# JediZ/PDE-based-image-processing

Measured on AMD Instinct MI355X. Metric: SOR iterations/sec (3840x2160 flow), higher is better.
Workload: dtype f32

## Files before the change

pde-based-image-processing_amd/csrc/pdeip_ctx.hip:

```cpp
#include "pdeip_ctx.hpp"

namespace pdeip {

Context g;
thread_local ThreadState tls;

int set_err(int code, const char *fmt, ...)
{
    va_list ap;
    va_start(ap, fmt);
    vsnprintf(tls.err, sizeof tls.err, fmt, ap);
    va_end(ap);
    return code;
}

SweepTimer::SweepTimer(hipStream_t stream) : s(stream)
{
    if (!g.profile) return;
    std::lock_guard<std::mutex> lock(g.ev_mutex);
    if (g.n_ev >= Context::MAX_EV) return;
    if (g.n_ev == g.n_ev_created) {
        if (hipEventCreate(&g.ev[g.n_ev][0]) != hipSuccess || hipEventCreate(&g.ev[g.n_ev][1]) != hipSuccess) return;
        g.n_ev_created++;
    }
    slot = g.n_ev++;
    (void)hipEventRecord(g.ev[slot][0], s);
}
void SweepTimer::stop(int launches)
{
    if (slot < 0) return;
    (void)hipEventRecord(g.ev[slot][1], s);
    g.ev_launches[slot] = launches;
}

static void latch_abort(DeviceState *d)
{
    if (!d->ws[WS_CTL] || !d->persist_used) return;
    unsigned word = 0;
    if (hipDeviceSynchronize() == hipSuccess && hipMemcpy(&word, d->ws[WS_CTL], sizeof word, hipMemcpyDeviceToHost) == hipSuccess && word != 0)
        d->abort_latched = true;
}

DeviceState *cur_dev()
{
    if (tls.dev_slot >= 0 && tls.dev_slot < MAX_DEVICES) return &g.devs[tls.dev_slot];
    int dev = 0;
// ... 306 lines not shown
```

pde-based-image-processing_amd/csrc/pdeip_ctx.hpp:

```cpp
#pragma once
#include "../../include/pdeip.h"

#include <hip/hip_runtime.h>

#include <atomic>
#include <cstdarg>
#include <cstdio>
#include <cstdlib>
#include <cstring>
#include <map>
#include <mutex>
#include <vector>

namespace pdeip {

enum { WS_AUX0 = 0, WS_AUX1, WS_PING, WS_ARENA, WS_CTL, WS_ORDER, WS_ALR, WS_ALR_T, WS_TV, WS_SMALL, WS_MAIL, WS_PACK, WS_DRIVER, WS_LEX, WS_LS, WS_NSLOT };

constexpr int MAX_DEVICES = 16;

struct DeviceState {
    int device = -1;
    void *ws[WS_NSLOT] = {};
    size_t ws_bytes[WS_NSLOT] = {};
    int order_B = 0, order_T = 0, order_affine = -1;
    int num_cus = 0;
    bool persist_used = false;
    bool abort_latched = false;
    std::map<const void *, size_t> lds_opt_in;
    std::map<const void *, int> resident_waves;
    hipStream_t worker_stream = nullptr;
    void reset_caches()
    {
        order_B = order_T = 0;
        order_affine = -1;
        persist_used = false;
    }
};

struct ThreadState {
    char err[512] = "";
    int last_launches = 0;
    int dev_slot = -1;
};
extern thread_local ThreadState tls;

struct Context {
    int mode = PDEIP_MODE_EXACT_ORDER;
    std::atomic<int> ws_generation{0};
    int rb_tj = 0;
    bool env_read = false;
    int ngroup = 1;
    int group[MAX_DEVICES] = {0};
    DeviceState devs[MAX_DEVICES];
    bool profile = false;
    static constexpr int MAX_EV = 4096;
    hipEvent_t ev[MAX_EV][2];
    int ev_launches[MAX_EV];
// ... 12 lines not shown

#define RC(expr)             \
    do {                     \
        int rc_ = (expr);    \
        if (rc_) return rc_; \
    } while (0)

#define NONNULL(who, p)                                                                                \
    do {                                                                                               \
        if ((p) == nullptr) return ::pdeip::set_err(PDEIP_ERR_ARG, "%s: argument '%s' is NULL", who, #p); \
    } while (0)

struct SweepTimer {
    hipStream_t s;
    int slot = -1;
    explicit SweepTimer(hipStream_t stream);
    void stop(int launches);
};

DeviceState *cur_dev();
int ws_get(int slot, size_t bytes, float **out);
int ensure_lds(const void *kernel, size_t bytes);
int resident_waves(const void *kernel, int block_threads, int waves_per_block);

int check_dims(const char *who, int nrows, int ncols, int nframes);
int check_mode(const char *who, int mode);
int check_solver(const char *who, int solver);
inline bool aligned16(const void *p) { return (reinterpret_cast<uintptr_t>(p) & 15u) == 0; }
int env_int(const char *name, int dflt);
int check_deriv_dims(const char *who, int nrows, int ncols, int nframes);
int pick_rb_tj(int nrows, int ncols);
int copy_d2d(hipStream_t s, float *dst, const float *src, size_t n);
inline dim3 pixel_grid(int nrows, int ncols, int nz) { return dim3((unsigned)((nrows + 255) / 256), (unsigned)ncols, (unsigned)nz); }
// ... 23 lines not shown
```

pde-based-image-processing_amd/csrc/pdeip_line.hip:

```cpp
#include "pdeip_ctx.hpp"

#include "pdeip_alr.hpp"

using namespace pdeip;

static int check_alr_line(const char *, int, int, int) { return PDEIP_OK; }

struct AlrFactors {
    float *cp[2][2], *dv[2][2];
};

template <class Mdl, bool VERT, int MODE>
static int zebra3_launch(hipStream_t s, const typename Mdl::Ctx &q, float *x, float *cp, float *dv, float *dp, int nrows, int ncols, int nframes,
                         int first, int lastc, int lstep, float omega)
{
    RC(ensure_lds(reinterpret_cast<const void *>(&k_alr_zebra3<Mdl, VERT, MODE>), Z3_LDS_BYTES));
    const int count = (lastc - first) / lstep + 1;
    hipLaunchKernelGGL((k_alr_zebra3<Mdl, VERT, MODE>), dim3((unsigned)((count + ZB_LW - 1) / ZB_LW), (unsigned)nframes), dim3(ZB_THREADS),
                       Z3_LDS_BYTES, s, q, x, cp, dv, dp, nrows, ncols, (size_t)nrows * ncols, first, lastc, lstep, omega);
    tls.last_launches++;
    HIPCHK(hipGetLastError());
    return PDEIP_OK;
}

template <class Mdl>
static int alr_factor(hipStream_t s, const typename Mdl::Ctx *q, const typename Mdl::Ctx *qt, int nch, int nrows, int ncols, int nframes,
                      AlrFactors *f)
{
    const size_t fs = (size_t)nrows * ncols, plane = fs * nframes;
    float *base;
    RC(ws_get(WS_ALR, plane * 8 * sizeof(float), &base));
    const int lo = Mdl::INTERIOR_LINES ? 1 : 0;
    for (int c = 0; c < nch; c++)
// ... 30 lines not shown
static int alr_lex_pass(hipStream_t s, const typename Mdl::Ctx *q, float *const *x, const AlrFactors &f, const int *order,
                        int nch, int nrows, int ncols, int nframes, bool vertical, float omega)
{
    const int lo = Mdl::INTERIOR_LINES ? 1 : 0;
    const int hi = (vertical ? ncols : nrows) - 1 - lo;
    const int n = vertical ? nrows : ncols;
    const size_t fs = (size_t)nrows * ncols;
    const int d = vertical ? 0 : 1;
    const size_t line_bytes = (size_t)n * sizeof(float4);
    if (line_bytes > 160 * 1024) {
        float *g = nullptr;
        RC(ws_get(WS_LEX, line_bytes * nframes, &g));
        for (int c = 0; c < nch; c++) {
            AlrChains<Mdl, 1> ch;
            ch.c[0] = AlrChain<Mdl>{q[order[c]], x[order[c]], f.cp[order[c]][d], f.dv[order[c]][d]};
            if (vertical) hipLaunchKernelGGL((k_alr_lex<Mdl, 1, true, true>), dim3((unsigned)nframes), dim3(ALR_LEX_THREADS), 0, s, ch, nrows, ncols, fs, lo, hi, omega, reinterpret_cast<float4 *>(g));
            else hipLaunchKernelGGL((k_alr_lex<Mdl, 1, false, true>), dim3((unsigned)nframes), dim3(ALR_LEX_THREADS), 0, s, ch, nrows, ncols, fs, lo, hi, omega, reinterpret_cast<float4 *>(g));
            tls.last_launches++;
        }
        HIPCHK(hipGetLastError());
        return PDEIP_OK;
    }
    if (nch == 2 && 2 * line_bytes <= 160 * 1024) {
        AlrChains<Mdl, 2> ch;
        for (int c = 0; c < 2; c++) ch.c[c] = AlrChain<Mdl>{q[order[c]], x[order[c]], f.cp[order[c]][d], f.dv[order[c]][d]};
        if (2 * line_bytes > 64 * 1024)
            RC(ensure_lds(vertical ? reinterpret_cast<const void *>(&k_alr_lex<Mdl, 2, true>) : reinterpret_cast<const void *>(&k_alr_lex<Mdl, 2, false>), 2 * line_bytes));
        if (vertical) hipLaunchKernelGGL((k_alr_lex<Mdl, 2, true>), dim3((unsigned)nframes), dim3(ALR_LEX_THREADS), 2 * line_bytes, s, ch, nrows, ncols, fs, lo, hi, omega);
        else hipLaunchKernelGGL((k_alr_lex<Mdl, 2, false>), dim3((unsigned)nframes), dim3(ALR_LEX_THREADS), 2 * line_bytes, s, ch, nrows, ncols, fs, lo, hi, omega);
        tls.last_launches++;
    } else {
        if (line_bytes > 64 * 1024)
            RC(ensure_lds(vertical ? reinterpret_cast<const void *>(&k_alr_lex<Mdl, 1, true>) : reinterpret_cast<const void *>(&k_alr_lex<Mdl, 1, false>), line_bytes));
        for (int c = 0; c < nch; c++) {
            AlrChains<Mdl, 1> ch;
            ch.c[0] = AlrChain<Mdl>{q[order[c]], x[order[c]], f.cp[order[c]][d], f.dv[order[c]][d]};
            if (vertical) hipLaunchKernelGGL((k_alr_lex<Mdl, 1, true>), dim3((unsigned)nframes), dim3(ALR_LEX_THREADS), line_bytes, s, ch, nrows, ncols, fs, lo, hi, omega);
            else hipLaunchKernelGGL((k_alr_lex<Mdl, 1, false>), dim3((unsigned)nframes), dim3(ALR_LEX_THREADS), line_bytes, s, ch, nrows, ncols, fs, lo, hi, omega);
            tls.last_launches++;
        }
    }
    HIPCHK(hipGetLastError());
    return PDEIP_OK;
}

template <class Mdl>
static int alr_zebra_pass(hipStream_t s, const typename Mdl::Ctx &q, float *x, const float *cpf, const float *dvf, int nrows, int ncols,
                          int nframes, bool vertical, float omega)
{
    const int lo = Mdl::INTERIOR_LINES ? 1 : 0;
    const int hi = (vertical ? ncols : nrows) - 1 - lo;
    const size_t fs = (size_t)nrows * ncols;
    float *cp, *dp;
    RC(ws_get(WS_AUX0, fs * nframes * sizeof(float), &cp));
    RC(ws_get(WS_AUX1, fs * nframes * sizeof(float), &dp));
    for (int colour = 0; colour < 2; colour++) {
        const int first = lo + (((lo & 1) != colour) ? 1 : 0);
        if (first > hi) continue;
        const int lastc = hi - (((hi & 1) != colour) ? 1 : 0);
        {
            if (cpf) {
                if (vertical) RC((zebra3_launch<Mdl, true, ZB_APPLY>(s, q, x, const_cast<float *>(cpf), const_cast<float *>(dvf), dp, nrows, ncols, nframes, first, lastc, 2, omega)));
                else RC((zebra3_launch<Mdl, false, ZB_APPLY>(s, q, x, const_cast<float *>(cpf), const_cast<float *>(dvf), dp, nrows, ncols, nframes, first, lastc, 2, omega)));
                continue;
            }
        }
        const int count = (hi - first) / 2 + 1;
        const dim3 grid((unsigned)((count + 63) / 64), (unsigned)nframes);
        if (vertical) hipLaunchKernelGGL((k_alr_zebra<Mdl, true>), grid, dim3(64), 0, s, q, x, cp, dp, nrows, ncols, fs, lo, hi, colour, omega);
        else hipLaunchKernelGGL((k_alr_zebra<Mdl, false>), grid, dim3(64), 0, s, q, x, cp, dp, nrows, ncols, fs, lo, hi, colour, omega);
        tls.last_launches++;
    }
    HIPCHK(hipGetLastError());
    return PDEIP_OK;
}

template <class Mdl>
static int alr_zebra_pass_pair(hipStream_t s, const typename Mdl::Ctx &qa, float *xa, const float *cpa, const float *dva, const typename Mdl::Ctx &qb,
                               float *xb, const float *cpb, const float *dvb, int nrows, int ncols, int nframes, bool vertical, float omega)
{
    const int lo = Mdl::INTERIOR_LINES ? 1 : 0;
    const int hi = (vertical ? ncols : nrows) - 1 - lo;
    const size_t fs = (size_t)nrows * ncols;
    float *dp;
    RC(ws_get(WS_AUX1, fs * nframes * sizeof(float), &dp));
    if (vertical) RC(ensure_lds(reinterpret_cast<const void *>(&k_alr_zebra3_pair<Mdl, true, ZB_APPLY>), Z3_LDS_BYTES));
    else RC(ensure_lds(reinterpret_cast<const void *>(&k_alr_zebra3_pair<Mdl, false, ZB_APPLY>), Z3_LDS_BYTES));
    for (int colour = 0; colour < 2; colour++) {
        const int first = lo + (((lo & 1) != colour) ? 1 : 0);
        if (first > hi) continue;
        const int lastc = hi - (((hi & 1) != colour) ? 1 : 0);
        const int count = (lastc - first) / 2 + 1;
        const dim3 grid((unsigned)((count + ZB_LW - 1) / ZB_LW), (unsigned)nframes);
        if (vertical)
            hipLaunchKernelGGL((k_alr_zebra3_pair<Mdl, true, ZB_APPLY>), grid, dim3(ZB_THREADS), Z3_LDS_BYTES, s, qa, xa, const_cast<float *>(cpa), const_cast<float *>(dva), qb, xb,
                               const_cast<float *>(cpb), const_cast<float *>(dvb), dp, nrows, ncols, fs, first, lastc, 2, omega);
        else
            hipLaunchKernelGGL((k_alr_zebra3_pair<Mdl, false, ZB_APPLY>), grid, dim3(ZB_THREADS), Z3_LDS_BYTES, s, qa, xa, const_cast<float *>(cpa), const_cast<float *>(dva), qb, xb,
                               const_cast<float *>(cpb), const_cast<float *>(dvb), dp, nrows, ncols, fs, first, lastc, 2, omega);
        tls.last_launches++;
    }
    HIPCHK(hipGetLastError());
    return PDEIP_OK;
}

struct AlrTwin {
    static constexpr int MAXP = 40;
    const float *orig[MAXP];
    float *twin[MAXP];
    int count = 0;
    float *find(const float *p) const
    {
        for (int k = 0; k < count; k++)
// ... 107 lines not shown
                    A.tin[k] = tin[k];
                    A.tout[k] = tout[k];
                }
                float *fbase;
                const size_t fplane = (size_t)nrows * ncols * nframes;
                RC(ws_get(WS_ALR, fplane * 8 * sizeof(float), &fbase));
                for (int c = 0; c < nch; c++)
                    for (int d = 0; d < 2; d++) {
                        A.cp[c][d] = fbase + fplane * (size_t)((c * 2 + d) * 2);
                        A.dv[c][d] = A.cp[c][d] + fplane;
                    }
                A.ntr = ntr; A.nch = nch; A.nrows = nrows; A.ncols = ncols; A.iter = iter; A.omega = omega;
                A.fs = (size_t)nrows * ncols;
                RC(ensure_lds(reinterpret_cast<const void *>(&k_alr_small<Mdl>), lds));
                SweepTimer timer(s);
                hipLaunchKernelGGL(k_alr_small<Mdl>, dim3((unsigned)nframes), dim3(ALR_SMALL_THREADS), lds, s, A);
                timer.stop(iter);
                tls.last_launches++;
                HIPCHK(hipGetLastError());
                return PDEIP_OK;
            }
            tw = AlrTwin{};
        }
    }
    RC(alr_make_twins(s, q, qt, nch, x, xt, nrows, ncols, nframes, &tw));
    AlrFactors f{};
    static const bool zebra1 = env_int("PDEIP_ALR_ZEBRA1", 0) != 0;
    if (mode == PDEIP_MODE_EXACT_ORDER || !zebra1) RC(alr_factor<Mdl>(s, q, qt, nch, nrows, ncols, nframes, &f));
    const bool pair = mode != PDEIP_MODE_EXACT_ORDER && nch == 2 && f.cp[0][0] != nullptr && f.cp[1][0] != nullptr && env_int("PDEIP_ALR_PAIR", 1) != 0;
    SweepTimer timer(s);
    for (int it = 0; it < iter; it++) {
// ... 81 lines not shown
```

pde-based-image-processing_amd/csrc/pdeip_sor5.hip:

```cpp
#include "pdeip_ctx.hpp"

#include "pdeip_models.hpp"
#include "pdeip_pointwise.hpp"
#include "pdeip_sor_exact.hpp"
#include "pdeip_walk_host.hpp"
#include "pdeip_persist_host.hpp"
#include "pdeip_sor_rb.hpp"
#include "pdeip_sor_rbp.hpp"
#include "pdeip_sor_small.hpp"

using namespace pdeip;

namespace {

template <class Mdl>
int pick_rb2_tj(int nrows, int ncols, int nframes, int ntiles_r)
{
    (void)nrows;
    const int forced = g.rb_tj > 0 ? g.rb_tj : env_int("PDEIP_RB_TJ", 0);
    if (forced > 0) return forced < 2 ? 2 : forced;
    const int slots = resident_waves(reinterpret_cast<const void *>(&k_sor_rb<Mdl, true, false, true>), 64 * RB_WAVES_PER_BLOCK, RB_WAVES_PER_BLOCK);
    int best = 12;
    long best_cost = -1;
    for (int tj = 2; tj <= 64; tj++) {
// ... 81 lines not shown
            RC(ws_get(WS_PACK, n * nframes * Mdl::NCF * sizeof(float), &pack));
            hipLaunchKernelGGL(k_pack_coefficients<Mdl>, pixel_grid(nrows, ncols, nframes), dim3(256), 0, s, P, pack, nrows, ncols, n);
            tls.last_launches++;
            const int NC = (nrows - 2 + 63 + EX_CH - 1) / EX_CH;
            const bool walk = env_int("PDEIP_EXACT_WALK", 0) != 0;
            const int W = walk ? walk_width<Mdl>(nrows, ncols, nframes, iter) : 64;
            const int BW = (ncols - 2 + W - 1) / W;
            PersistCtl ctl{};
            RC(persist_prepare(s, BW, iter, nframes, (size_t)nframes * iter * BW * NIT * (size_t)NC * EX_CH * sizeof(unsigned long long), &ctl));
            SweepTimer timer(s);
            if (walk) {
                RC(walk_launch<Mdl>(s, P, pack, ctl, nrows, ncols, BW, iter, NC, nframes, omega, n, W));
            } else {
                constexpr size_t plds = ExactLayout<Mdl>::LDS_BYTES + 16;
                RC(ensure_lds(reinterpret_cast<const void *>(&k_sor_exact_persist<Mdl>), plds));
                hipLaunchKernelGGL(k_sor_exact_persist<Mdl>, dim3((unsigned)(BW * iter * nframes)), dim3(exp_threads<Mdl>()), plds, s, P, pack, ctl, nrows, ncols, BW, iter, NC, nframes, omega, n);
            }
            timer.stop(1);
            tls.last_launches++;
            const int nb = 2 * ncols + 2 * (nrows - 2);
            hipLaunchKernelGGL(k_fill_borders, dim3((nb + 255) / 256, nframes, NIT), dim3(256), 0, s,
                               P.it_out[0], P.it_out[NIT - 1], NIT, nrows, ncols, n);
            tls.last_launches++;
            HIPCHK(hipGetLastError());
            return PDEIP_OK;
        }
        hipLaunchKernelGGL(k_derive<Mdl>, pixel_grid(nrows, ncols, nframes), dim3(256), 0, s, P, aux0, aux1, nrows, ncols, n);
        tls.last_launches++;
        P.cf[Mdl::D0] = aux0;
        P.cf[Mdl::D1] = aux1;
        const dim3 grid((unsigned)(B * iter), (unsigned)nframes);
        constexpr size_t lds = ExactLayout<Mdl>::LDS_BYTES;
        RC(ensure_lds(reinterpret_cast<const void *>(&k_sor_exact<Mdl>), lds));
        SweepTimer timer(s);
        for (int m = 0; m <= last_m; m++) {
            hipLaunchKernelGGL(k_sor_exact<Mdl>, grid, dim3(128), lds, s, P, nrows, ncols, A, B, iter, m, omega, n);
            tls.last_launches++;
        }
        timer.stop(last_m + 1);
        const int nb = 2 * ncols + 2 * (nrows - 2);
        hipLaunchKernelGGL(k_fill_borders, dim3((nb + 255) / 256, nframes, NIT), dim3(256), 0, s,
                           P.it_out[0], P.it_out[NIT - 1], NIT, nrows, ncols, n);
        tls.last_launches++;
        HIPCHK(hipGetLastError());
        return PDEIP_OK;
    }

    const bool small_enabled = env_int("PDEIP_RB_SMALL", 1) != 0;
    if (small_enabled) {
        using SL = SmallLayout<Mdl>;
        const int qpref = env_int("PDEIP_SMALL_Q", 1);
// ... 20 lines not shown
                counter = reinterpret_cast<unsigned *>(p);
                RC(ws_get(WS_CTL, 16, &p));
                abort_word = reinterpret_cast<unsigned *>(p);
            }
            DeviceState *d = cur_dev();
            for (int f = 0; f < NIT; f++) {
                P.it_in[f] = P.it_out[f];
                if (dst) P.it_out[f] = dst[f];
            }
            SweepTimer timer(s);
            int nl = 0;
            for (int it = 0; it < iter; it += per_launch, nl++) {
                const int k = iter - it < per_launch ? iter - it : per_launch;
                const bool gated = sp.nslabs > 1 && P.it_in[0] == P.it_out[0];
                if (gated) d->persist_used = true;
                hipLaunchKernelGGL(k_sor_small<Mdl>, dim3((unsigned)sp.nslabs, (unsigned)nframes), dim3(SL::THREADS), sp.lds, s, P, nrows, ncols, k,
                                   omega, col0, n, sp.W, gated ? counter : nullptr, abort_word);
                for (int f = 0; f < NIT; f++) P.it_in[f] = P.it_out[f];
            }
            timer.stop(nl);
            tls.last_launches += nl;
            HIPCHK(hipGetLastError());
            return PDEIP_OK;
        }
    }

    float *scratch = nullptr;
    int rc = ws_get(WS_PING, (size_t)NIT * n * nframes * sizeof(float), &scratch);
    if (rc) return rc;
    float *bufA[NIT], *bufB[NIT], *bufD[NIT];
    bool vec = (nrows % 4 == 0);
// ... 33 lines not shown
            using PL = RbpLayout<Mdl, PS>;
            const bool first = it == 0;
            const void *kfn = first ? reinterpret_cast<const void *>(&k_sor_rbp<Mdl, PS, true>) : reinterpret_cast<const void *>(&k_sor_rbp<Mdl, PS, false>);
            RC(ensure_lds(kfn, PL::LDS_BYTES));
            const int ntiles_p = (nrows + RBP_OWN_ROWS - 1) / RBP_OWN_ROWS;
            const int TJP = pick_rbp_tj<Mdl, PS>(ncols, nframes, ntiles_p, kfn);
            const int nunits = ntiles_p * ((ncols + TJP - 1) / TJP);
            for (int f = 0; f < NIT; f++) {
                P.it_in[f] = buf_in(flips, f);
                P.it_out[f] = buf_out(flips, f);
            }
            const bool keep = first && it + PS < iter;
            const dim3 pgrid((unsigned)nunits, (unsigned)nframes), pblock(PL::THREADS);
            const int serp = env_int("PDEIP_RBP_SERPENTINE", 0);
            const int mirror_mode = serp < 0 || serp > 2 ? 0 : serp;
            if (first) hipLaunchKernelGGL((k_sor_rbp<Mdl, PS, true>), pgrid, pblock, PL::LDS_BYTES, s, P, keep ? aux0 : nullptr, keep ? aux1 : nullptr, nrows, ncols, TJP, ntiles_p, nunits, omega, col0, n, mirror_mode);
            else hipLaunchKernelGGL((k_sor_rbp<Mdl, PS, false>), pgrid, pblock, PL::LDS_BYTES, s, P, nullptr, nullptr, nrows, ncols, TJP, ntiles_p, nunits, omega, col0, n, mirror_mode);
            if (first) {
                P.cf[Mdl::D0] = aux0;
                P.cf[Mdl::D1] = aux1;
            }
            it += PS;
            flips++;
            nlaunch++;
            tls.last_launches++;
            continue;
        }
        const bool two = fuse && it + 2 <= iter;
        const int TJ = two ? TJ2 : TJ1;
        const int nunits = ntiles_r * ((ncols + TJ - 1) / TJ);
        const dim3 grid((unsigned)((nunits + RB_WAVES_PER_BLOCK - 1) / RB_WAVES_PER_BLOCK), (unsigned)nframes);
        for (int f = 0; f < NIT; f++) {
            P.it_in[f] = buf_in(flips, f);
            P.it_out[f] = buf_out(flips, f);
        }
        const bool first = it == 0;
        float *d0 = first ? aux0 : nullptr, *d1 = first ? aux1 : nullptr;
#define PDEIP_RB_LAUNCH(V, F, T) hipLaunchKernelGGL((k_sor_rb<Mdl, V, F, T>), grid, block, 0, s, P, d0, d1, nrows, ncols, TJ, ntiles_r, nunits, omega, col0, n)
        if (two) {
            if (vec) { if (first) PDEIP_RB_LAUNCH(true, true, true); else PDEIP_RB_LAUNCH(true, false, true); }
            else     { if (first) PDEIP_RB_LAUNCH(false, true, true); else PDEIP_RB_LAUNCH(false, false, true); }
        } else {
            if (vec) { if (first) PDEIP_RB_LAUNCH(true, true, false); else PDEIP_RB_LAUNCH(true, false, false); }
            else     { if (first) PDEIP_RB_LAUNCH(false, true, false); else PDEIP_RB_LAUNCH(false, false, false); }
        }
#undef PDEIP_RB_LAUNCH
        if (first) {
            P.cf[Mdl::D0] = aux0;
            P.cf[Mdl::D1] = aux1;
        }
        it += two ? 2 : 1;
        flips++;
        nlaunch++;
// ... 222 lines not shown
```

pde-based-image-processing_amd/csrc/pdeip_sor9.hip:

```cpp
#include "pdeip_ctx.hpp"

#include "pdeip_models.hpp"
#include "pdeip_pointwise.hpp"
#include "pdeip_sor_pde8.hpp"
#include "pdeip_sor_pde8_persist.hpp"
#include "pdeip_persist_host.hpp"
#include <vector>
#include "pdeip_sor_rb.hpp"

using namespace pdeip;

extern "C" int pdeip_pde_sor8_dev(void *stream, float *X, const float *TRACE, const float *B, const float *wW,
                                  const float *wNW, const float *wN, const float *wNE, const float *wE,
                                  const float *wSE, const float *wS, const float *wSW, int nrows, int ncols,
                                  int nframes, int iter, float omega, int mode, int col0)
{
    const char *who = "pdeip_pde_sor8_dev";
    RC(check_dims(who, nrows, ncols, nframes));
    RC(check_mode(who, mode));
    hipStream_t s = static_cast<hipStream_t>(stream);
    tls.last_launches = 0;
    if (iter <= 0) return PDEIP_OK;
    const size_t n = (size_t)nrows * ncols, nf = n * (size_t)nframes;
    float *bt, *inv, *scratch = nullptr;
// ... 62 lines not shown
                    TJ2 = tj;
                }
            }
        }
    }
    SweepTimer timer(s);
    int nlaunch = 0, flips = 0;
    for (int it = 0; it < iter;) {
        const bool two = fuse && it + 2 <= iter, first = it == 0;
        const int TJ = two ? TJ2 : TJ1, ntiles_r = two ? ntiles2 : ntiles1;
        const int nunits = ntiles_r * ((ncols + TJ - 1) / TJ);
        const dim3 grid((unsigned)((nunits + RB_WAVES_PER_BLOCK - 1) / RB_WAVES_PER_BLOCK), (unsigned)nframes);
        P.x_in = (flips & 1) ? scratch : X;
        P.x_out = (flips & 1) ? X : scratch;
        float *d0 = first ? bt : nullptr, *d1 = first ? inv : nullptr;
#define PDEIP_P8_LAUNCH(KERNEL, V, F) hipLaunchKernelGGL((KERNEL<V, F>), grid, block, 0, s, P, d0, d1, nrows, ncols, TJ, ntiles_r, nunits, omega, col0, n)
        if (two) {
            if (vec) { if (first) PDEIP_P8_LAUNCH(k_pde8_colour2, true, true); else PDEIP_P8_LAUNCH(k_pde8_colour2, true, false); }
            else     { if (first) PDEIP_P8_LAUNCH(k_pde8_colour2, false, true); else PDEIP_P8_LAUNCH(k_pde8_colour2, false, false); }
        } else {
            if (vec) { if (first) PDEIP_P8_LAUNCH(k_pde8_colour, true, true); else PDEIP_P8_LAUNCH(k_pde8_colour, true, false); }
            else     { if (first) PDEIP_P8_LAUNCH(k_pde8_colour, false, true); else PDEIP_P8_LAUNCH(k_pde8_colour, false, false); }
        }
#undef PDEIP_P8_LAUNCH
        if (first) {
            P.cf[ModelPde8::cB] = bt;
            P.cf[ModelPde8::cInv] = inv;
        }
        it += two ? 2 : 1;
        flips++;
        nlaunch++;
// ... 17 lines not shown
```

pde-based-image-processing_amd/csrc/pdeip_sor_pde8.hpp:

```cpp
#pragma once
#include "pdeip_models.hpp"
#include "pdeip_sor_exact.hpp"
#include "pdeip_sor_rb.hpp"

namespace pdeip {

struct Pde8Planes {
    float *x;
    const float *cf[ModelPde8::NCF];
};


template <int E0>
__device__ __forceinline__ void p8_phase(float (&C)[4], const float (&W)[4], const float (&E)[4],
                                         const float (&cf)[ModelPde8::NCF][4], int r, int nrows, float omega, float om1)
{
    const float ce = (E0 == 0) ? lane_above(C[3]) : lane_below(C[0]);
    const float we = (E0 == 0) ? lane_above(W[3]) : lane_below(W[0]);
    const float ee = (E0 == 0) ? lane_above(E[3]) : lane_below(E[0]);
#pragma unroll
    for (int e = E0; e < 4; e += 2) {
        const int i = r + e;
        if (i >= 1 && i <= nrows - 2) {
            const int em = e == 0 ? 0 : e - 1, ep = e == 3 ? 3 : e + 1;
// ... 566 lines not shown
        lds_barrier();
    }
}

inline int pde8_run_exact(hipStream_t s, Pde8Planes P, float *side, int nrows, int ncols, int nframes,
                          int iter, float omega)
{
    const size_t n = (size_t)nrows * ncols;
    const int A = (nrows - 2 + P8_SKEW * 63 + P8_R - 1) / P8_R;
    const int B = (ncols - 2 + 63) / 64;
    const int last_m = (A - 1) + P8_G * (B - 1) + P8_H * (iter - 1);
    const dim3 grid((unsigned)(B * iter), (unsigned)nframes);
    if (ensure_lds(reinterpret_cast<const void *>(&k_pde8_exact), Pde8Layout::LDS_BYTES) != PDEIP_OK) return -1;
    int launches = 0;
    for (int m = 0; m <= last_m; m++) {
        hipLaunchKernelGGL(k_pde8_exact, grid, dim3(128), Pde8Layout::LDS_BYTES, s, P, side, nrows, ncols, A, B, iter, m, omega, n);
        launches++;
    }
    const int nb = 2 * ncols + 2 * (nrows - 2);
    hipLaunchKernelGGL(k_fill_borders, dim3((nb + 255) / 256, nframes, 1), dim3(256), 0, s, P.x, P.x, 1, nrows, ncols, n);
    return launches + 1;
}

}
```

pde-based-image-processing_amd/csrc/pdeip_sor_pde8_persist.hpp:

```cpp
#pragma once
#include "pdeip_sor_pde8.hpp"

namespace pdeip {

constexpr int P8P_THREADS = 256;

__host__ __device__ inline int pde8_pack_blocks(int nrows) { return (nrows + 2) / 2; }
inline size_t pde8_pack_floats(int nrows, int ncols, int nframes) { return (size_t)pde8_pack_blocks(nrows) * ncols * 2 * ModelPde8::NCF * nframes; }

static __global__ void k_pde8_pack(float *pack, const float *TRACE, const float *B, const float *wW, const float *wNW, const float *wN,
                                   const float *wNE, const float *wE, const float *wSE, const float *wS, const float *wSW, int nrows,
                                   int ncols, size_t frame_stride)
{
    constexpr int NCF = ModelPde8::NCF;
    const int nb = pde8_pack_blocks(nrows);
    const int pb = blockIdx.x * blockDim.x + threadIdx.x, col = ncols - 1 - (int)blockIdx.y;
    if (pb >= nb) return;
    const size_t fo = (size_t)blockIdx.z * frame_stride;
    float v[NCF][2];
#pragma unroll
    for (int r2 = 0; r2 < 2; r2++) {
        const int row = 2 * pb + r2 - 1;
        const bool in = row >= 0 && row < nrows;
        const size_t p = fo + (size_t)col * nrows + (in ? row : 0);
// ... 374 lines not shown
        }
        P8S_END;
        lds_barrier();
    }
    P8S_WRITE;
}

inline int pde8_run_exact_persist(hipStream_t s, Pde8Planes P, const float *pack, float *side, PersistCtl ctl, int nrows, int ncols, int nframes, int iter,
                                  float omega)
{
    const size_t n = (size_t)nrows * ncols;
    const int B = (ncols - 2 + 63) / 64;
    const int NC = pde8_persist_chunks(nrows);
    constexpr size_t lds = Pde8Layout::LDS_BYTES + 16;
    if (ensure_lds(reinterpret_cast<const void *>(&k_pde8_exact_persist), lds) != PDEIP_OK) return -1;
    hipLaunchKernelGGL(k_pde8_exact_persist, dim3((unsigned)(B * iter * nframes)), dim3(P8P_THREADS), lds, s, P, pack, side, ctl, nrows, ncols, B, iter,
                       NC, nframes, omega, n);
    const int nb = 2 * ncols + 2 * (nrows - 2);
    hipLaunchKernelGGL(k_fill_borders, dim3((nb + 255) / 256, nframes, 1), dim3(256), 0, s, P.x, P.x, 1, nrows, ncols, n);
    return 2;
}

}
```

pde-based-image-processing_amd/csrc/pdeip_sor_rbp.hpp:

```cpp
#pragma once
#include "pdeip_sor_rb.hpp"

namespace pdeip {

constexpr int RBP_OWN_ROWS = 240;

template <class Mdl, int S> struct RbpLayout {
    static constexpr int NIT = Mdl::NIT, NRO = Mdl::NRO, NCF = Mdl::NCF;
    static constexpr int NRING = NCF + NRO;
    static constexpr int COL = 256;
    static constexpr int GROUP = NRING + NIT;
#ifndef RBP_NK_SLACK
#define RBP_NK_SLACK 1
#endif
    static constexpr int nk_for(int p) { return p + 3 * (S - 1) + RBP_NK_SLACK; }
    static constexpr int nq_for(int p) { return NRO > 0 ? p + 3 * (S - 1) + 1 : 0; }
    static constexpr size_t lds_for(int p)
    {
        return (size_t)(nk_for(p) * NCF * COL + nq_for(p) * NRO * COL + (p + 1) * NIT * COL + (S - 1) * 2 * NIT * COL) * sizeof(float);
    }
    static constexpr int pick_lead()
    {
        int best = 0;
        for (int p = 1; p <= 8; p++)
// ... 11 lines not shown
    static constexpr int K_FLOATS = NK * NCF * COL;
    static constexpr int Q_FLOATS = nq_for(P) * NRO * COL;
    static constexpr int O_FLOATS = NO * NIT * COL;
    static constexpr int H_FLOATS = (S - 1) * 2 * NIT * COL;
    static constexpr size_t LDS_BYTES = (size_t)(K_FLOATS + Q_FLOATS + O_FLOATS + H_FLOATS) * sizeof(float);
    static constexpr int NW = (NIT == 2) ? 2 : 1;
#ifndef RBP_LOADERS
#define RBP_LOADERS 1
#endif
    static constexpr int NLOAD = RBP_LOADERS;
    static constexpr int THREADS = 64 * (S * NW + NLOAD);
    static constexpr int pieces_of(int w) { return (GROUP - w + NLOAD - 1) / NLOAD; }
    static constexpr int HALO = 2 * S;
    static constexpr bool FITS = P >= 2 && LDS_BYTES <= 160 * 1024 && (P - 1) * GROUP <= 63;
    __host__ __device__ static constexpr int nsteps(int tj) { return tj + 5 * S - 1; }
};

typedef float rbp_f4 __attribute__((ext_vector_type(4)));
typedef __attribute__((address_space(3))) rbp_f4 rbp_lds_f4;
__device__ __forceinline__ void rbp_lds_read(float (&d)[4], const float *col, int lane)
{
    const rbp_f4 t = *(const rbp_lds_f4 *)(col + 4 * lane);
    d[0] = t.x; d[1] = t.y; d[2] = t.z; d[3] = t.w;
}
__device__ __forceinline__ void rbp_lds_write(float *col, int lane, const float (&d)[4])
{
    const rbp_f4 t = {d[0], d[1], d[2], d[3]};
    *(rbp_lds_f4 *)(col + 4 * lane) = t;
}

// ... 377 lines not shown
                if (L::NLOAD == 1 || (NCF + f) % L::NLOAD == lw)
                    __builtin_amdgcn_global_load_lds(RBP_GLB(P.ro[f] + off), RBP_LDS(qdst + f * COL), 16, 0, 0);
            float *odst = Oring + (size_t)oslot * NIT * COL;
#pragma unroll
            for (int f = 0; f < NIT; f++)
                if (L::NLOAD == 1 || (NCF + NRO + f) % L::NLOAD == lw)
                    __builtin_amdgcn_global_load_lds(RBP_GLB(P.it_in[f] + off), RBP_LDS(odst + f * COL), 16, 0, 0);
            kslot = (kslot + 1 == L::NK) ? 0 : kslot + 1;
            qslot = (qslot + 1 == L::NQ) ? 0 : qslot + 1;
            oslot = (oslot + 1 == L::NO) ? 0 : oslot + 1;
        };
        auto landed = [&]() __attribute__((always_inline)) {
            if (lw == 0) asm volatile("s_waitcnt vmcnt(%0)" ::"n"((L::P - 1) * L::pieces_of(0)) : "memory");
            else asm volatile("s_waitcnt vmcnt(%0)" ::"n"((L::P - 1) * L::pieces_of(L::NLOAD > 1 ? 1 : 0)) : "memory");
        };
        static_assert(L::NLOAD == 1 || L::NLOAD == 2, "one or two loader waves");
        for (int g = 0; g < L::P; g++) issue(g);
        landed();
        rbp_barrier();
#ifndef RBP_LOADER_SLEEP
#define RBP_LOADER_SLEEP 0
#endif
        for (int t = 0; t < nsteps; t++) {
#ifdef PDEIP_RBP_STAMPS
            const bool stamp_on = (blockIdx.x == 100) && (RBP_STAMP_SWEEP == 9) && (lw == 0) && (t >= RBP_STAMP_T0) && (t < RBP_STAMP_T0 + 24);
#endif
            RBP_STAMP(0);
            if (RBP_LOADER_SLEEP > 0) __builtin_amdgcn_s_sleep(RBP_LOADER_SLEEP);
            if (t + L::P < nsteps) {
                issue(t + L::P);
                RBP_STAMP(1);
                landed();
            } else {
                asm volatile("s_waitcnt vmcnt(0)" ::: "memory");
            }
            RBP_STAMP(2);
            RBP_STAMP(3);
            RBP_STAMP(4);
            rbp_barrier();
            RBP_STAMP(5);
        }
        asm volatile("s_waitcnt vmcnt(0)" ::: "memory");
        return;
    }

#ifndef RBP_ROLE_REMAP
#define RBP_ROLE_REMAP 1
#endif
    if constexpr (NW == 2) {
// ... 13 lines not shown
```

pde-based-image-processing_amd/csrc/pdeip_walk5.hip:

```cpp
#include "pdeip_walk_host.hpp"

#include "pdeip_sor_walk.hpp"

namespace pdeip {

template <class Mdl> int walk_width(int nrows, int ncols, int nframes, int iter)
{
    (void)nrows; (void)ncols; (void)nframes; (void)iter;
    const int forced = env_int("PDEIP_WALK_W", 0);
    if (forced == 32 || forced == 48 || forced == 64) return forced;
    return 64;
}

namespace {
template <class Mdl, int NBUF, int W>
int launch_one(hipStream_t s, const SweepPlanes<Mdl> &P, const float *pack, const PersistCtl &ctl, int nrows, int ncols, int B, int iter, int NC,
               int nframes, float omega, size_t n)
{
    using WL = WalkLayout<Mdl, NBUF, W>;
    static_assert(WL::FITS, "the chunk buffers must fit the 160 KB of LDS");
    RC(ensure_lds(reinterpret_cast<const void *>(&k_sor_walk<Mdl, NBUF, W>), WL::LDS_BYTES));
    hipLaunchKernelGGL((k_sor_walk<Mdl, NBUF, W>), dim3((unsigned)(B * iter * nframes)), dim3(WL::THREADS), WL::LDS_BYTES, s, P, pack, ctl, nrows, ncols, B,
                       iter, NC, nframes, omega, n, env_int("PDEIP_WALK_TUNE", 0));
    return PDEIP_OK;
}
template <class Mdl, int W>
int launch_w(hipStream_t s, const SweepPlanes<Mdl> &P, const float *pack, const PersistCtl &ctl, int nrows, int ncols, int B, int iter, int NC,
             int nframes, float omega, size_t n)
{
    constexpr int NB = WalkLayout<Mdl, 3, W>::FITS ? 3 : 2;
    if (NB == 3 && env_int("PDEIP_WALK_NBUF", 3) < 3) return launch_one<Mdl, 2, W>(s, P, pack, ctl, nrows, ncols, B, iter, NC, nframes, omega, n);
    return launch_one<Mdl, NB, W>(s, P, pack, ctl, nrows, ncols, B, iter, NC, nframes, omega, n);
}
}

template <class Mdl>
int walk_launch(hipStream_t s, const SweepPlanes<Mdl> &P, const float *pack, const PersistCtl &ctl, int nrows, int ncols, int B, int iter, int NC,
// ... 33 lines not shown
```

Before: 35000.

## Time sweeps with launch-attached events and refine RBP loader tail waits

Replaces separate hipEventRecord calls around sweeps with hipExtLaunchKernelGGL start/stop events attached to the first and last kernels. It also changes the red-black pipelined kernel's loader loop to stop issuing at the real group count instead of the step count. The tail then waits only for the outstanding group it needs rather than draining all loads with vmcnt(0). The timing change only matters when profiling is enabled. The tail change lets loader waves overlap the final groups, at the cost of more intricate waitcnt bookkeeping.

Result: faster. 35800, median of 5 (+2.3%).

```diff
diff --git a/pde-based-image-processing_amd/csrc/pdeip_ctx.hip b/pde-based-image-processing_amd/csrc/pdeip_ctx.hip
--- a/pde-based-image-processing_amd/csrc/pdeip_ctx.hip
+++ b/pde-based-image-processing_amd/csrc/pdeip_ctx.hip
@@ -16,7 +16,7 @@
 
 SweepTimer::SweepTimer(hipStream_t stream) : s(stream)
 {
-    if (!g.profile) return;
+    if (!g.profile || tls.timer != nullptr) return;
     std::lock_guard<std::mutex> lock(g.ev_mutex);
     if (g.n_ev >= Context::MAX_EV) return;
     if (g.n_ev == g.n_ev_created) {
@@ -24,12 +24,20 @@
         g.n_ev_created++;
     }
     slot = g.n_ev++;
-    (void)hipEventRecord(g.ev[slot][0], s);
+    g.ev_launches[slot] = 0;
+    tls.timer = this;
+}
+SweepTimer::~SweepTimer()
+{
+    if (tls.timer == this) tls.timer = nullptr;
 }
 void SweepTimer::stop(int launches)
 {
     if (slot < 0) return;
-    (void)hipEventRecord(g.ev[slot][1], s);
+    if (tls.timer == this) tls.timer = nullptr;
+    if (!started) (void)hipEventRecord(g.ev[slot][0], s);
+    if (!stopped) (void)hipEventRecord(g.ev[slot][1], s);
+    started = stopped = true;
     g.ev_launches[slot] = launches;
 }
 
diff --git a/pde-based-image-processing_amd/csrc/pdeip_ctx.hpp b/pde-based-image-processing_amd/csrc/pdeip_ctx.hpp
--- a/pde-based-image-processing_amd/csrc/pdeip_ctx.hpp
+++ b/pde-based-image-processing_amd/csrc/pdeip_ctx.hpp
@@ -2,6 +2,7 @@
 #include "../../include/pdeip.h"
 
 #include <hip/hip_runtime.h>
+#include <hip/hip_ext.h>
 
 #include <atomic>
 #include <cstdarg>
@@ -37,10 +38,12 @@
     }
 };
 
+struct SweepTimer;
 struct ThreadState {
     char err[512] = "";
     int last_launches = 0;
     int dev_slot = -1;
+    SweepTimer *timer = nullptr;
 };
 extern thread_local ThreadState tls;
 
@@ -83,9 +86,29 @@
 struct SweepTimer {
     hipStream_t s;
     int slot = -1;
+    bool started = false, stopped = false;
     explicit SweepTimer(hipStream_t stream);
+    ~SweepTimer();
+    SweepTimer(const SweepTimer &) = delete;
+    SweepTimer &operator=(const SweepTimer &) = delete;
     void stop(int launches);
 };
+
+template <class... K, class... A>
+inline void sweep_launch(bool last, void (*kernel)(K...), dim3 grid, dim3 block, size_t lds, hipStream_t s, A &&...args)
+{
+    static_assert(sizeof...(K) == sizeof...(A), "one argument per kernel parameter");
+    SweepTimer *t = tls.timer;
+    const bool first = t != nullptr && !t->started;
+    if (t == nullptr || !(first || last)) {
+        hipLaunchKernelGGL(kernel, grid, block, lds, s, static_cast<K>(args)...);
+        return;
+    }
+    hipExtLaunchKernelGGL(kernel, grid, block, (uint32_t)lds, s, first ? g.ev[t->slot][0] : nullptr, last ? g.ev[t->slot][1] : nullptr, 0,
+                          static_cast<K>(args)...);
+    t->started = true;
+    t->stopped = t->stopped || last;
+}
 
 DeviceState *cur_dev();
 int ws_get(int slot, size_t bytes, float **out);
diff --git a/pde-based-image-processing_amd/csrc/pdeip_line.hip b/pde-based-image-processing_amd/csrc/pdeip_line.hip
--- a/pde-based-image-processing_amd/csrc/pdeip_line.hip
+++ b/pde-based-image-processing_amd/csrc/pdeip_line.hip
@@ -16,7 +16,7 @@
 {
     RC(ensure_lds(reinterpret_cast<const void *>(&k_alr_zebra3<Mdl, VERT, MODE>), Z3_LDS_BYTES));
     const int count = (lastc - first) / lstep + 1;
-    hipLaunchKernelGGL((k_alr_zebra3<Mdl, VERT, MODE>), dim3((unsigned)((count + ZB_LW - 1) / ZB_LW), (unsigned)nframes), dim3(ZB_THREADS),
+    sweep_launch(false, k_alr_zebra3<Mdl, VERT, MODE>, dim3((unsigned)((count + ZB_LW - 1) / ZB_LW), (unsigned)nframes), dim3(ZB_THREADS),
                        Z3_LDS_BYTES, s, q, x, cp, dv, dp, nrows, ncols, (size_t)nrows * ncols, first, lastc, lstep, omega);
     tls.last_launches++;
     HIPCHK(hipGetLastError());
@@ -77,8 +77,8 @@
         for (int c = 0; c < nch; c++) {
             AlrChains<Mdl, 1> ch;
             ch.c[0] = AlrChain<Mdl>{q[order[c]], x[order[c]], f.cp[order[c]][d], f.dv[order[c]][d]};
-            if (vertical) hipLaunchKernelGGL((k_alr_lex<Mdl, 1, true, true>), dim3((unsigned)nframes), dim3(ALR_LEX_THREADS), 0, s, ch, nrows, ncols, fs, lo, hi, omega, reinterpret_cast<float4 *>(g));
-            else hipLaunchKernelGGL((k_alr_lex<Mdl, 1, false, true>), dim3((unsigned)nframes), dim3(ALR_LEX_THREADS), 0, s, ch, nrows, ncols, fs, lo, hi, omega, reinterpret_cast<float4 *>(g));
+            if (vertical) sweep_launch(false, k_alr_lex<Mdl, 1, true, true>, dim3((unsigned)nframes), dim3(ALR_LEX_THREADS), 0, s, ch, nrows, ncols, fs, lo, hi, omega, reinterpret_cast<float4 *>(g));
+            else sweep_launch(false, k_alr_lex<Mdl, 1, false, true>, dim3((unsigned)nframes), dim3(ALR_LEX_THREADS), 0, s, ch, nrows, ncols, fs, lo, hi, omega, reinterpret_cast<float4 *>(g));
             tls.last_launches++;
         }
         HIPCHK(hipGetLastError());
@@ -89,8 +89,8 @@
         for (int c = 0; c < 2; c++) ch.c[c] = AlrChain<Mdl>{q[order[c]], x[order[c]], f.cp[order[c]][d], f.dv[order[c]][d]};
         if (2 * line_bytes > 64 * 1024)
             RC(ensure_lds(vertical ? reinterpret_cast<const void *>(&k_alr_lex<Mdl, 2, true>) : reinterpret_cast<const void *>(&k_alr_lex<Mdl, 2, false>), 2 * line_bytes));
-        if (vertical) hipLaunchKernelGGL((k_alr_lex<Mdl, 2, true>), dim3((unsigned)nframes), dim3(ALR_LEX_THREADS), 2 * line_bytes, s, ch, nrows, ncols, fs, lo, hi, omega);
-        else hipLaunchKernelGGL((k_alr_lex<Mdl, 2, false>), dim3((unsigned)nframes), dim3(ALR_LEX_THREADS), 2 * line_bytes, s, ch, nrows, ncols, fs, lo, hi, omega);
+        if (vertical) sweep_launch(false, k_alr_lex<Mdl, 2, true>, dim3((unsigned)nframes), dim3(ALR_LEX_THREADS), 2 * line_bytes, s, ch, nrows, ncols, fs, lo, hi, omega, nullptr);
+        else sweep_launch(false, k_alr_lex<Mdl, 2, false>, dim3((unsigned)nframes), dim3(ALR_LEX_THREADS), 2 * line_bytes, s, ch, nrows, ncols, fs, lo, hi, omega, nullptr);
         tls.last_launches++;
     } else {
         if (line_bytes > 64 * 1024)
@@ -98,8 +98,8 @@
         for (int c = 0; c < nch; c++) {
             AlrChains<Mdl, 1> ch;
             ch.c[0] = AlrChain<Mdl>{q[order[c]], x[order[c]], f.cp[order[c]][d], f.dv[order[c]][d]};
-            if (vertical) hipLaunchKernelGGL((k_alr_lex<Mdl, 1, true>), dim3((unsigned)nframes), dim3(ALR_LEX_THREADS), line_bytes, s, ch, nrows, ncols, fs, lo, hi, omega);
-            else hipLaunchKernelGGL((k_alr_lex<Mdl, 1, false>), dim3((unsigned)nframes), dim3(ALR_LEX_THREADS), line_bytes, s, ch, nrows, ncols, fs, lo, hi, omega);
+            if (vertical) sweep_launch(false, k_alr_lex<Mdl, 1, true>, dim3((unsigned)nframes), dim3(ALR_LEX_THREADS), line_bytes, s, ch, nrows, ncols, fs, lo, hi, omega, nullptr);
+            else sweep_launch(false, k_alr_lex<Mdl, 1, false>, dim3((unsigned)nframes), dim3(ALR_LEX_THREADS), line_bytes, s, ch, nrows, ncols, fs, lo, hi, omega, nullptr);
             tls.last_launches++;
         }
     }
@@ -130,8 +130,8 @@
         }
         const int count = (hi - first) / 2 + 1;
         const dim3 grid((unsigned)((count + 63) / 64), (unsigned)nframes);
-        if (vertical) hipLaunchKernelGGL((k_alr_zebra<Mdl, true>), grid, dim3(64), 0, s, q, x, cp, dp, nrows, ncols, fs, lo, hi, colour, omega);
-        else hipLaunchKernelGGL((k_alr_zebra<Mdl, false>), grid, dim3(64), 0, s, q, x, cp, dp, nrows, ncols, fs, lo, hi, colour, omega);
+        if (vertical) sweep_launch(false, k_alr_zebra<Mdl, true>, grid, dim3(64), 0, s, q, x, cp, dp, nrows, ncols, fs, lo, hi, colour, omega);
+        else sweep_launch(false, k_alr_zebra<Mdl, false>, grid, dim3(64), 0, s, q, x, cp, dp, nrows, ncols, fs, lo, hi, colour, omega);
         tls.last_launches++;
     }
     HIPCHK(hipGetLastError());
@@ -156,10 +156,10 @@
         const int count = (lastc - first) / 2 + 1;
         const dim3 grid((unsigned)((count + ZB_LW - 1) / ZB_LW), (unsigned)nframes);
         if (vertical)
-            hipLaunchKernelGGL((k_alr_zebra3_pair<Mdl, true, ZB_APPLY>), grid, dim3(ZB_THREADS), Z3_LDS_BYTES, s, qa, xa, const_cast<float *>(cpa), const_cast<float *>(dva), qb, xb,
+            sweep_launch(false, k_alr_zebra3_pair<Mdl, true, ZB_APPLY>, grid, dim3(ZB_THREADS), Z3_LDS_BYTES, s, qa, xa, const_cast<float *>(cpa), const_cast<float *>(dva), qb, xb,
                                const_cast<float *>(cpb), const_cast<float *>(dvb), dp, nrows, ncols, fs, first, lastc, 2, omega);
         else
-            hipLaunchKernelGGL((k_alr_zebra3_pair<Mdl, false, ZB_APPLY>), grid, dim3(ZB_THREADS), Z3_LDS_BYTES, s, qa, xa, const_cast<float *>(cpa), const_cast<float *>(dva), qb, xb,
+            sweep_launch(false, k_alr_zebra3_pair<Mdl, false, ZB_APPLY>, grid, dim3(ZB_THREADS), Z3_LDS_BYTES, s, qa, xa, const_cast<float *>(cpa), const_cast<float *>(dva), qb, xb,
                                const_cast<float *>(cpb), const_cast<float *>(dvb), dp, nrows, ncols, fs, first, lastc, 2, omega);
         tls.last_launches++;
     }
@@ -297,7 +297,7 @@
                 A.fs = (size_t)nrows * ncols;
                 RC(ensure_lds(reinterpret_cast<const void *>(&k_alr_small<Mdl>), lds));
                 SweepTimer timer(s);
-                hipLaunchKernelGGL(k_alr_small<Mdl>, dim3((unsigned)nframes), dim3(ALR_SMALL_THREADS), lds, s, A);
+                sweep_launch(true, k_alr_small<Mdl>, dim3((unsigned)nframes), dim3(ALR_SMALL_THREADS), lds, s, A);
                 timer.stop(iter);
                 tls.last_launches++;
                 HIPCHK(hipGetLastError());
diff --git a/pde-based-image-processing_amd/csrc/pdeip_sor5.hip b/pde-based-image-processing_amd/csrc/pdeip_sor5.hip
--- a/pde-based-image-processing_amd/csrc/pdeip_sor5.hip
+++ b/pde-based-image-processing_amd/csrc/pdeip_sor5.hip
@@ -119,7 +119,7 @@
             } else {
                 constexpr size_t plds = ExactLayout<Mdl>::LDS_BYTES + 16;
                 RC(ensure_lds(reinterpret_cast<const void *>(&k_sor_exact_persist<Mdl>), plds));
-                hipLaunchKernelGGL(k_sor_exact_persist<Mdl>, dim3((unsigned)(BW * iter * nframes)), dim3(exp_threads<Mdl>()), plds, s, P, pack, ctl, nrows, ncols, BW, iter, NC, nframes, omega, n);
+                sweep_launch(true, k_sor_exact_persist<Mdl>, dim3((unsigned)(BW * iter * nframes)), dim3(exp_threads<Mdl>()), plds, s, P, pack, ctl, nrows, ncols, BW, iter, NC, nframes, omega, n);
             }
             timer.stop(1);
             tls.last_launches++;
@@ -139,7 +139,7 @@
         RC(ensure_lds(reinterpret_cast<const void *>(&k_sor_exact<Mdl>), lds));
         SweepTimer timer(s);
         for (int m = 0; m <= last_m; m++) {
-            hipLaunchKernelGGL(k_sor_exact<Mdl>, grid, dim3(128), lds, s, P, nrows, ncols, A, B, iter, m, omega, n);
+            sweep_launch(m == last_m, k_sor_exact<Mdl>, grid, dim3(128), lds, s, P, nrows, ncols, A, B, iter, m, omega, n);
             tls.last_launches++;
         }
         timer.stop(last_m + 1);
@@ -190,7 +190,7 @@
                 const int k = iter - it < per_launch ? iter - it : per_launch;
                 const bool gated = sp.nslabs > 1 && P.it_in[0] == P.it_out[0];
                 if (gated) d->persist_used = true;
-                hipLaunchKernelGGL(k_sor_small<Mdl>, dim3((unsigned)sp.nslabs, (unsigned)nframes), dim3(SL::THREADS), sp.lds, s, P, nrows, ncols, k,
+                sweep_launch(it + per_launch >= iter, k_sor_small<Mdl>, dim3((unsigned)sp.nslabs, (unsigned)nframes), dim3(SL::THREADS), sp.lds, s, P, nrows, ncols, k,
                                    omega, col0, n, sp.W, gated ? counter : nullptr, abort_word);
                 for (int f = 0; f < NIT; f++) P.it_in[f] = P.it_out[f];
             }
@@ -254,8 +254,9 @@
             const dim3 pgrid((unsigned)nunits, (unsigned)nframes), pblock(PL::THREADS);
             const int serp = env_int("PDEIP_RBP_SERPENTINE", 0);
             const int mirror_mode = serp < 0 || serp > 2 ? 0 : serp;
-            if (first) hipLaunchKernelGGL((k_sor_rbp<Mdl, PS, true>), pgrid, pblock, PL::LDS_BYTES, s, P, keep ? aux0 : nullptr, keep ? aux1 : nullptr, nrows, ncols, TJP, ntiles_p, nunits, omega, col0, n, mirror_mode);
-            else hipLaunchKernelGGL((k_sor_rbp<Mdl, PS, false>), pgrid, pblock, PL::LDS_BYTES, s, P, nullptr, nullptr, nrows, ncols, TJP, ntiles_p, nunits, omega, col0, n, mirror_mode);
+            const bool last = nlaunch + 1 == total_launches;
+            if (first) sweep_launch(last, k_sor_rbp<Mdl, PS, true>, pgrid, pblock, PL::LDS_BYTES, s, P, keep ? aux0 : nullptr, keep ? aux1 : nullptr, nrows, ncols, TJP, ntiles_p, nunits, omega, col0, n, mirror_mode);
+            else sweep_launch(last, k_sor_rbp<Mdl, PS, false>, pgrid, pblock, PL::LDS_BYTES, s, P, nullptr, nullptr, nrows, ncols, TJP, ntiles_p, nunits, omega, col0, n, mirror_mode);
             if (first) {
                 P.cf[Mdl::D0] = aux0;
                 P.cf[Mdl::D1] = aux1;
@@ -276,7 +277,7 @@
         }
         const bool first = it == 0;
         float *d0 = first ? aux0 : nullptr, *d1 = first ? aux1 : nullptr;
-#define PDEIP_RB_LAUNCH(V, F, T) hipLaunchKernelGGL((k_sor_rb<Mdl, V, F, T>), grid, block, 0, s, P, d0, d1, nrows, ncols, TJ, ntiles_r, nunits, omega, col0, n)
+#define PDEIP_RB_LAUNCH(V, F, T) sweep_launch(nlaunch + 1 == total_launches, k_sor_rb<Mdl, V, F, T>, grid, block, 0, s, P, d0, d1, nrows, ncols, TJ, ntiles_r, nunits, omega, col0, n)
         if (two) {
             if (vec) { if (first) PDEIP_RB_LAUNCH(true, true, true); else PDEIP_RB_LAUNCH(true, false, true); }
             else     { if (first) PDEIP_RB_LAUNCH(false, true, true); else PDEIP_RB_LAUNCH(false, false, true); }
diff --git a/pde-based-image-processing_amd/csrc/pdeip_sor9.hip b/pde-based-image-processing_amd/csrc/pdeip_sor9.hip
--- a/pde-based-image-processing_amd/csrc/pdeip_sor9.hip
+++ b/pde-based-image-processing_amd/csrc/pdeip_sor9.hip
@@ -100,7 +100,7 @@
         P.x_in = (flips & 1) ? scratch : X;
         P.x_out = (flips & 1) ? X : scratch;
         float *d0 = first ? bt : nullptr, *d1 = first ? inv : nullptr;
-#define PDEIP_P8_LAUNCH(KERNEL, V, F) hipLaunchKernelGGL((KERNEL<V, F>), grid, block, 0, s, P, d0, d1, nrows, ncols, TJ, ntiles_r, nunits, omega, col0, n)
+#define PDEIP_P8_LAUNCH(KERNEL, V, F) sweep_launch(it + (two ? 2 : 1) >= iter, KERNEL<V, F>, grid, block, 0, s, P, d0, d1, nrows, ncols, TJ, ntiles_r, nunits, omega, col0, n)
         if (two) {
             if (vec) { if (first) PDEIP_P8_LAUNCH(k_pde8_colour2, true, true); else PDEIP_P8_LAUNCH(k_pde8_colour2, true, false); }
             else     { if (first) PDEIP_P8_LAUNCH(k_pde8_colour2, false, true); else PDEIP_P8_LAUNCH(k_pde8_colour2, false, false); }
diff --git a/pde-based-image-processing_amd/csrc/pdeip_sor_pde8.hpp b/pde-based-image-processing_amd/csrc/pdeip_sor_pde8.hpp
--- a/pde-based-image-processing_amd/csrc/pdeip_sor_pde8.hpp
+++ b/pde-based-image-processing_amd/csrc/pdeip_sor_pde8.hpp
@@ -604,11 +604,11 @@
     if (ensure_lds(reinterpret_cast<const void *>(&k_pde8_exact), Pde8Layout::LDS_BYTES) != PDEIP_OK) return -1;
     int launches = 0;
     for (int m = 0; m <= last_m; m++) {
-        hipLaunchKernelGGL(k_pde8_exact, grid, dim3(128), Pde8Layout::LDS_BYTES, s, P, side, nrows, ncols, A, B, iter, m, omega, n);
+        sweep_launch(false, k_pde8_exact, grid, dim3(128), Pde8Layout::LDS_BYTES, s, P, side, nrows, ncols, A, B, iter, m, omega, n);
         launches++;
     }
     const int nb = 2 * ncols + 2 * (nrows - 2);
-    hipLaunchKernelGGL(k_fill_borders, dim3((nb + 255) / 256, nframes, 1), dim3(256), 0, s, P.x, P.x, 1, nrows, ncols, n);
+    sweep_launch(true, k_fill_borders, dim3((nb + 255) / 256, nframes, 1), dim3(256), 0, s, P.x, P.x, 1, nrows, ncols, n);
     return launches + 1;
 }
 
diff --git a/pde-based-image-processing_amd/csrc/pdeip_sor_pde8_persist.hpp b/pde-based-image-processing_amd/csrc/pdeip_sor_pde8_persist.hpp
--- a/pde-based-image-processing_amd/csrc/pdeip_sor_pde8_persist.hpp
+++ b/pde-based-image-processing_amd/csrc/pdeip_sor_pde8_persist.hpp
@@ -412,10 +412,10 @@
     const int NC = pde8_persist_chunks(nrows);
     constexpr size_t lds = Pde8Layout::LDS_BYTES + 16;
     if (ensure_lds(reinterpret_cast<const void *>(&k_pde8_exact_persist), lds) != PDEIP_OK) return -1;
-    hipLaunchKernelGGL(k_pde8_exact_persist, dim3((unsigned)(B * iter * nframes)), dim3(P8P_THREADS), lds, s, P, pack, side, ctl, nrows, ncols, B, iter,
+    sweep_launch(false, k_pde8_exact_persist, dim3((unsigned)(B * iter * nframes)), dim3(P8P_THREADS), lds, s, P, pack, side, ctl, nrows, ncols, B, iter,
                        NC, nframes, omega, n);
     const int nb = 2 * ncols + 2 * (nrows - 2);
-    hipLaunchKernelGGL(k_fill_borders, dim3((nb + 255) / 256, nframes, 1), dim3(256), 0, s, P.x, P.x, 1, nrows, ncols, n);
+    sweep_launch(true, k_fill_borders, dim3((nb + 255) / 256, nframes, 1), dim3(256), 0, s, P.x, P.x, 1, nrows, ncols, n);
     return 2;
 }
 
diff --git a/pde-based-image-processing_amd/csrc/pdeip_sor_rbp.hpp b/pde-based-image-processing_amd/csrc/pdeip_sor_rbp.hpp
--- a/pde-based-image-processing_amd/csrc/pdeip_sor_rbp.hpp
+++ b/pde-based-image-processing_amd/csrc/pdeip_sor_rbp.hpp
@@ -49,6 +49,7 @@
     static constexpr int HALO = 2 * S;
     static constexpr bool FITS = P >= 2 && LDS_BYTES <= 160 * 1024 && (P - 1) * GROUP <= 63;
     __host__ __device__ static constexpr int nsteps(int tj) { return tj + 5 * S - 1; }
+    __host__ __device__ static constexpr int ngroups(int tj) { return tj + 4 * S; }
 };
 
 typedef float rbp_f4 __attribute__((ext_vector_type(4)));
@@ -456,7 +457,17 @@
             if (lw == 0) asm volatile("s_waitcnt vmcnt(%0)" ::"n"((L::P - 1) * L::pieces_of(0)) : "memory");
             else asm volatile("s_waitcnt vmcnt(%0)" ::"n"((L::P - 1) * L::pieces_of(L::NLOAD > 1 ? 1 : 0)) : "memory");
         };
+        auto landed_tail = [&](int k) __attribute__((always_inline)) {
+#define PDEIP_RBP_TAIL(N) case N: asm volatile("s_waitcnt vmcnt(%0)" ::"n"((N) * L::GROUP <= 63 ? (N) * L::GROUP : 0) : "memory"); break;
+            switch (L::NLOAD == 1 && k < L::P - 1 ? L::P - 1 - k : 0) {
+                PDEIP_RBP_TAIL(1) PDEIP_RBP_TAIL(2) PDEIP_RBP_TAIL(3) PDEIP_RBP_TAIL(4) PDEIP_RBP_TAIL(5) PDEIP_RBP_TAIL(6)
+            default: asm volatile("s_waitcnt vmcnt(0)" ::: "memory"); break;
+            }
+#undef PDEIP_RBP_TAIL
+        };
         static_assert(L::NLOAD == 1 || L::NLOAD == 2, "one or two loader waves");
+        static_assert(L::P <= 8, "landed_tail() counts down from P - 2 <= 6 groups in flight");
+        const int ngroups = L::ngroups(TJ);
         for (int g = 0; g < L::P; g++) issue(g);
         landed();
         rbp_barrier();
@@ -469,12 +480,12 @@
 #endif
             RBP_STAMP(0);
             if (RBP_LOADER_SLEEP > 0) __builtin_amdgcn_s_sleep(RBP_LOADER_SLEEP);
-            if (t + L::P < nsteps) {
+            if (t + L::P < ngroups) {
                 issue(t + L::P);
                 RBP_STAMP(1);
                 landed();
             } else {
-                asm volatile("s_waitcnt vmcnt(0)" ::: "memory");
+                landed_tail(t + L::P - (ngroups - 1));
             }
             RBP_STAMP(2);
             RBP_STAMP(3);
diff --git a/pde-based-image-processing_amd/csrc/pdeip_walk5.hip b/pde-based-image-processing_amd/csrc/pdeip_walk5.hip
--- a/pde-based-image-processing_amd/csrc/pdeip_walk5.hip
+++ b/pde-based-image-processing_amd/csrc/pdeip_walk5.hip
@@ -20,7 +20,7 @@
     using WL = WalkLayout<Mdl, NBUF, W>;
     static_assert(WL::FITS, "the chunk buffers must fit the 160 KB of LDS");
     RC(ensure_lds(reinterpret_cast<const void *>(&k_sor_walk<Mdl, NBUF, W>), WL::LDS_BYTES));
-    hipLaunchKernelGGL((k_sor_walk<Mdl, NBUF, W>), dim3((unsigned)(B * iter * nframes)), dim3(WL::THREADS), WL::LDS_BYTES, s, P, pack, ctl, nrows, ncols, B,
+    sweep_launch(true, k_sor_walk<Mdl, NBUF, W>, dim3((unsigned)(B * iter * nframes)), dim3(WL::THREADS), WL::LDS_BYTES, s, P, pack, ctl, nrows, ncols, B,
                        iter, NC, nframes, omega, n, env_int("PDEIP_WALK_TUNE", 0));
     return PDEIP_OK;
 }
```
